# valida-xyz/valida

Measured on NVIDIA H100. Metric: trace rows/sec proven (Fibonacci), higher is better.
Workload: dtype u32 (BabyBear, 31-bit modular) + ext5

## Files before the change

valida_b200/csrc/keccak.cuh:

```cuda
#pragma once
#include <cstdint>
#include <cuda_runtime.h>

namespace kk {

__constant__ uint2 RC[24] = {
    {0x00000001u, 0x00000000u}, {0x00008082u, 0x00000000u}, {0x0000808au, 0x80000000u}, {0x80008000u, 0x80000000u},
    {0x0000808bu, 0x00000000u}, {0x80000001u, 0x00000000u}, {0x80008081u, 0x80000000u}, {0x00008009u, 0x80000000u},
    {0x0000008au, 0x00000000u}, {0x00000088u, 0x00000000u}, {0x80008009u, 0x00000000u}, {0x8000000au, 0x00000000u},
    {0x8000808bu, 0x00000000u}, {0x0000008bu, 0x80000000u}, {0x00008089u, 0x80000000u}, {0x00008003u, 0x80000000u},
    {0x00008002u, 0x80000000u}, {0x00000080u, 0x80000000u}, {0x0000800au, 0x00000000u}, {0x8000000au, 0x80000000u},
    {0x80008081u, 0x80000000u}, {0x00008080u, 0x80000000u}, {0x80000001u, 0x00000000u}, {0x80008008u, 0x80000000u}};

__constant__ uint32_t POW2[32] = {1u << 0, 1u << 1, 1u << 2, 1u << 3, 1u << 4, 1u << 5, 1u << 6, 1u << 7, 1u << 8, 1u << 9, 1u << 10, 1u << 11,
                                  1u << 12, 1u << 13, 1u << 14, 1u << 15, 1u << 16, 1u << 17, 1u << 18, 1u << 19, 1u << 20, 1u << 21, 1u << 22,
                                  1u << 23, 1u << 24, 1u << 25, 1u << 26, 1u << 27, 1u << 28, 1u << 29, 1u << 30, 1u << 31};

template <int M> __device__ __forceinline__ uint2 rol_small(uint2 a) {
    const uint32_t p = POW2[M];
    uint32_t wlo, whi, nlo, nhi;
    asm("{\n\t.reg .u64 w;\n\tmul.wide.u32 w, %4, %6;\n\tmov.b64 {%0, %1}, w;\n\tmad.lo.u32 %3, %5, %6, %1;\n\tmad.hi.u32 %2, %5, %6, %0;\n\t}"
        : "=&r"(wlo), "=&r"(whi), "=r"(nlo), "=r"(nhi) : "r"(a.x), "r"(a.y), "r"(p));
    return make_uint2(nlo, nhi);
}
#ifndef KK_FMA_ROT_MASK
#define KK_FMA_ROT_MASK 0ull
#endif
template <int M> __device__ __forceinline__ uint2 rol_shf(uint2 a) {
    return make_uint2(__funnelshift_l(a.y, a.x, M), __funnelshift_l(a.x, a.y, M));
}
template <int N> __device__ __forceinline__ uint2 rol(uint2 a) {
    if (N == 0) return a;
    if (N == 32) return make_uint2(a.y, a.x);
    constexpr int M = (N & 31) ? (N & 31) : 1;
    const uint2 b = N < 32 ? a : make_uint2(a.y, a.x);
    if ((KK_FMA_ROT_MASK >> N) & 1ull) return rol_small<M>(b);
    return rol_shf<M>(b);
}
__device__ __forceinline__ uint2 x2(uint2 a, uint2 b) { return make_uint2(a.x ^ b.x, a.y ^ b.y); }
__device__ __forceinline__ uint2 x3(uint2 a, uint2 b, uint2 c) { return make_uint2(a.x ^ b.x ^ c.x, a.y ^ b.y ^ c.y); }
__device__ __forceinline__ uint2 x5(uint2 a, uint2 b, uint2 c, uint2 d, uint2 e) { return make_uint2(a.x ^ b.x ^ c.x ^ d.x ^ e.x, a.y ^ b.y ^ c.y ^ d.y ^ e.y); }
__device__ __forceinline__ uint2 chi(uint2 a, uint2 b, uint2 c) { return make_uint2(a.x ^ (~b.x & c.x), a.y ^ (~b.y & c.y)); }

__device__ __forceinline__ void keccak_round(uint2 A[25], const uint2 rc) {
    uint2 C0 = x5(A[0], A[5], A[10], A[15], A[20]);
    uint2 C1 = x5(A[1], A[6], A[11], A[16], A[21]);
    uint2 C2 = x5(A[2], A[7], A[12], A[17], A[22]);
    uint2 C3 = x5(A[3], A[8], A[13], A[18], A[23]);
    uint2 C4 = x5(A[4], A[9], A[14], A[19], A[24]);
    const uint2 R0 = rol<1>(C1), R1 = rol<1>(C2), R2 = rol<1>(C3), R3 = rol<1>(C4), R4 = rol<1>(C0);
    uint2 B0 = x3(A[0], C4, R0);
    uint2 B10 = rol<1>(x3(A[1], C0, R1));
    uint2 B20 = rol<62>(x3(A[2], C1, R2));
    uint2 B5 = rol<28>(x3(A[3], C2, R3));
    uint2 B15 = rol<27>(x3(A[4], C3, R4));
    uint2 B16 = rol<36>(x3(A[5], C4, R0));
    uint2 B1 = rol<44>(x3(A[6], C0, R1));
    uint2 B11 = rol<6>(x3(A[7], C1, R2));
    uint2 B21 = rol<55>(x3(A[8], C2, R3));
    uint2 B6 = rol<20>(x3(A[9], C3, R4));
    uint2 B7 = rol<3>(x3(A[10], C4, R0));
    uint2 B17 = rol<10>(x3(A[11], C0, R1));
    uint2 B2 = rol<43>(x3(A[12], C1, R2));
    uint2 B12 = rol<25>(x3(A[13], C2, R3));
    uint2 B22 = rol<39>(x3(A[14], C3, R4));
    uint2 B23 = rol<41>(x3(A[15], C4, R0));
    uint2 B8 = rol<45>(x3(A[16], C0, R1));
    uint2 B18 = rol<15>(x3(A[17], C1, R2));
    uint2 B3 = rol<21>(x3(A[18], C2, R3));
    uint2 B13 = rol<8>(x3(A[19], C3, R4));
    uint2 B14 = rol<18>(x3(A[20], C4, R0));
    uint2 B24 = rol<2>(x3(A[21], C0, R1));
    uint2 B9 = rol<61>(x3(A[22], C1, R2));
    uint2 B19 = rol<56>(x3(A[23], C2, R3));
    uint2 B4 = rol<14>(x3(A[24], C3, R4));
    A[0] = chi(B0, B1, B2); A[1] = chi(B1, B2, B3); A[2] = chi(B2, B3, B4); A[3] = chi(B3, B4, B0); A[4] = chi(B4, B0, B1);
    A[5] = chi(B5, B6, B7); A[6] = chi(B6, B7, B8); A[7] = chi(B7, B8, B9); A[8] = chi(B8, B9, B5); A[9] = chi(B9, B5, B6);
    A[10] = chi(B10, B11, B12); A[11] = chi(B11, B12, B13); A[12] = chi(B12, B13, B14); A[13] = chi(B13, B14, B10); A[14] = chi(B14, B10, B11);
    A[15] = chi(B15, B16, B17); A[16] = chi(B16, B17, B18); A[17] = chi(B17, B18, B19); A[18] = chi(B18, B19, B15); A[19] = chi(B19, B15, B16);
    A[20] = chi(B20, B21, B22); A[21] = chi(B21, B22, B23); A[22] = chi(B22, B23, B24); A[23] = chi(B23, B24, B20); A[24] = chi(B24, B20, B21);
    A[0].x ^= rc.x; A[0].y ^= rc.y;
}

template <bool FIRST, bool LAST>
__device__ __forceinline__ void keccak_f_peeled(uint2 A[25]) {
    if (FIRST) keccak_round(A, make_uint2(0x00000001u, 0x00000000u));
#pragma unroll 1
    for (int round = FIRST ? 1 : 0; round < (LAST ? 23 : 24); round++) keccak_round(A, RC[round]);
    if (LAST) keccak_round(A, make_uint2(0x80008008u, 0x80000000u));
}
__device__ __forceinline__ void keccak_f(uint2 A[25]) { keccak_f_peeled<false, false>(A); }

}
```

valida_b200/csrc/merkle.cu:

```cuda
#include "ctx.h"
#include "keccak.cuh"
#include "merkle.h"
#include <algorithm>
#include <cstdlib>
#include <numeric>

namespace {

constexpr int RATE_WORDS = 34;

template <bool SHORT = false, class Fetch>
__device__ __forceinline__ void keccak256_words(const uint32_t nwords, Fetch fetch, uint32_t out[8]) {
    uint2 A[25];
#pragma unroll
    for (int i = 0; i < 25; i++) A[i] = make_uint2(0, 0);
    uint32_t nblocks = nwords / RATE_WORDS + 1;
    if (SHORT) {
#pragma unroll
        for (int i = 0; i < RATE_WORDS / 2; i++) {
            const uint32_t g0 = 2 * i, g1 = g0 + 1;
            uint32_t w0 = g0 < nwords ? fetch(g0) : (g0 == nwords ? 1u : 0u);
            uint32_t w1 = g1 < nwords ? fetch(g1) : (g1 == nwords ? 1u : 0u);
            if (i == RATE_WORDS / 2 - 1) w1 ^= 0x80000000u;
            A[i] = make_uint2(w0, w1);
        }
        kk::keccak_f_peeled<true, true>(A);
        out[0] = A[0].x; out[1] = A[0].y; out[2] = A[1].x; out[3] = A[1].y;
        out[4] = A[2].x; out[5] = A[2].y; out[6] = A[3].x; out[7] = A[3].y;
        return;
    }
    for (uint32_t b = 0; b < nblocks; b++) {
        uint32_t base = b * RATE_WORDS;
#pragma unroll
        for (int i = 0; i < RATE_WORDS / 2; i++) {
            uint32_t g0 = base + 2 * i, g1 = g0 + 1;
            uint32_t w0 = g0 < nwords ? fetch(g0) : (g0 == nwords ? 1u : 0u);
            uint32_t w1 = g1 < nwords ? fetch(g1) : (g1 == nwords ? 1u : 0u);
            if (i == RATE_WORDS / 2 - 1 && b == nblocks - 1) w1 ^= 0x80000000u;
            A[i].x ^= w0; A[i].y ^= w1;
        }
        if (b == nblocks - 1) kk::keccak_f_peeled<false, true>(A); else kk::keccak_f(A);
    }
    out[0] = A[0].x; out[1] = A[0].y; out[2] = A[1].x; out[3] = A[1].y;
    out[4] = A[2].x; out[5] = A[2].y; out[6] = A[3].x; out[7] = A[3].y;
}

__device__ __forceinline__ uint32_t wrap_mod_p(uint32_t w) {
    w = bb::umin32(w, w - bb::P);
    return bb::umin32(w, w - bb::P);
}

__global__ void __launch_bounds__(128) leaf_hash_kernel(const uint32_t* const* __restrict__ colptr, uint32_t nwords, uint64_t row0, uint64_t nrows, uint32_t* __restrict__ digests) {
    uint64_t r = (uint64_t)blockIdx.x * blockDim.x + threadIdx.x;
    if (r >= nrows) return;
    r += row0;
    uint32_t d[8];
    keccak256_words(nwords, [&](uint32_t i) { return bb::from_monty(__ldg(colptr[i] + r)); }, d);
    uint4* o = reinterpret_cast<uint4*>(digests + r * 8);
    o[0] = make_uint4(wrap_mod_p(d[0]), wrap_mod_p(d[1]), wrap_mod_p(d[2]), wrap_mod_p(d[3]));
    o[1] = make_uint4(wrap_mod_p(d[4]), wrap_mod_p(d[5]), wrap_mod_p(d[6]), wrap_mod_p(d[7]));
}

__device__ __forceinline__ void compress_pair(const uint32_t l[8], const uint32_t r[8], uint32_t out[8]) {
    uint32_t d[8];
    keccak256_words<true>(16, [&](uint32_t i) { return i < 8 ? l[i] : r[i - 8]; }, d);
#pragma unroll
    for (int i = 0; i < 8; i++) out[i] = wrap_mod_p(d[i]);
}

__global__ void __launch_bounds__(128) compress_layer_kernel(const uint32_t* __restrict__ prev, const uint32_t* __restrict__ inject, uint64_t i0, uint64_t n_next, uint32_t* __restrict__ next) {
    uint64_t i = (uint64_t)blockIdx.x * blockDim.x + threadIdx.x;
    if (i >= n_next) return;
    i += i0;
    uint32_t l[8], r[8], o[8];
    const uint4* p = reinterpret_cast<const uint4*>(prev + i * 16);
    uint4 a = __ldg(p), b = __ldg(p + 1), c = __ldg(p + 2), d = __ldg(p + 3);
    l[0] = a.x; l[1] = a.y; l[2] = a.z; l[3] = a.w; l[4] = b.x; l[5] = b.y; l[6] = b.z; l[7] = b.w;
    r[0] = c.x; r[1] = c.y; r[2] = c.z; r[3] = c.w; r[4] = d.x; r[5] = d.y; r[6] = d.z; r[7] = d.w;
    compress_pair(l, r, o);
    if (inject) {
        const uint4* q = reinterpret_cast<const uint4*>(inject + i * 8);
        uint4 e = __ldg(q), f = __ldg(q + 1);
        uint32_t t[8] = {e.x, e.y, e.z, e.w, f.x, f.y, f.z, f.w};
        uint32_t o2[8];
        compress_pair(o, t, o2);
#pragma unroll
        for (int k = 0; k < 8; k++) o[k] = o2[k];
    }
    uint4* w = reinterpret_cast<uint4*>(next + i * 8);
    w[0] = make_uint4(o[0], o[1], o[2], o[3]);
    w[1] = make_uint4(o[4], o[5], o[6], o[7]);
}

__constant__ uint8_t WK_ROT[25] = {0, 1, 62, 28, 27, 36, 44, 6, 55, 20, 3, 10, 43, 25, 39, 41, 45, 15, 21, 8, 18, 2, 61, 56, 14};
struct WarpKeccak {
    uint32_t rot, col[4], dm, dp, pi, c1, c2, lane;
    __device__ __forceinline__ void init(uint32_t lane_) {
        lane = lane_;
        const uint32_t t = lane < 25 ? lane : 0, x = t % 5, y = t / 5;
        rot = WK_ROT[t];
#pragma unroll
        for (int k = 0; k < 4; k++) col[k] = (t + 5 * (k + 1)) % 25;
        dm = (x + 4) % 5 + 5 * y; dp = (x + 1) % 5 + 5 * y;
        pi = (x + 3 * y) % 5 + 5 * x;
        c1 = (x + 1) % 5 + 5 * y; c2 = (x + 2) % 5 + 5 * y;
    }
    static __device__ __forceinline__ uint2 sh(uint2 v, uint32_t src) { return make_uint2(__shfl_sync(0xffffffffu, v.x, src), __shfl_sync(0xffffffffu, v.y, src)); }
    __device__ __forceinline__ void permute(uint2& a) const {
#pragma unroll 1
        for (int round = 0; round < 24; round++) {
            uint2 p = a;
#pragma unroll
            for (int k = 0; k < 4; k++) { const uint2 o = sh(a, col[k]); p.x ^= o.x; p.y ^= o.y; }
            const uint2 pm = sh(p, dm), pp = sh(p, dp);
            a.x ^= pm.x ^ __funnelshift_l(pp.y, pp.x, 1); a.y ^= pm.y ^ __funnelshift_l(pp.x, pp.y, 1);
            uint32_t lo = a.x, hi = a.y;
            if (rot & 32) { const uint32_t tmp = lo; lo = hi; hi = tmp; }
            uint2 b = make_uint2(__funnelshift_l(hi, lo, rot & 31), __funnelshift_l(lo, hi, rot & 31));
            b = sh(b, pi);
            const uint2 b1 = sh(b, c1), b2 = sh(b, c2);
            a.x = b.x ^ (~b1.x & b2.x); a.y = b.y ^ (~b1.y & b2.y);
            if (lane == 0) { const uint2 rc = kk::RC[round]; a.x ^= rc.x; a.y ^= rc.y; }
            if (lane >= 25) a = make_uint2(0, 0);
        }
    }
    __device__ __forceinline__ uint2 compress(uint2 words) const {
        uint2 a = lane < 8 ? words : lane == 8 ? make_uint2(1u, 0u) : lane == 16 ? make_uint2(0u, 0x80000000u) : make_uint2(0u, 0u);
        permute(a);
        return make_uint2(wrap_mod_p(a.x), wrap_mod_p(a.y));
    }
};

constexpr int TAIL_SUB = 256, TAIL_THREADS = 512, TAIL_MAX_LEVELS = 9, TAIL_WARP_NODES = 32;
struct TailParams {
    const uint32_t* prev_v;
    uint32_t* next_v[TAIL_MAX_LEVELS];
    const uint32_t* inj_v[TAIL_MAX_LEVELS];
    uint64_t first_begin;
    uint32_t sub;
    uint32_t levels;
};
__global__ void __maxnreg__(80) tree_tail_kernel(const __grid_constant__ TailParams p) {
    __shared__ uint4 buf_a[2 * TAIL_SUB * 2];
    __shared__ uint4 buf_b[TAIL_SUB * 2];
    const uint64_t node0 = p.first_begin + (uint64_t)blockIdx.x * p.sub;
    {
        const uint4* src = reinterpret_cast<const uint4*>(p.prev_v + 2 * node0 * 8);
        for (uint32_t i = threadIdx.x; i < 4 * p.sub; i += TAIL_THREADS) buf_a[i] = __ldg(src + i);
    }
    __syncthreads();
    WarpKeccak wk;
    wk.init(threadIdx.x & 31);
    uint4* cur = buf_a; uint4* nxt = buf_b;
    for (uint32_t k = 0; k < p.levels; k++) {
        const uint32_t n = p.sub >> k;
        const uint64_t base = node0 >> k;
        if (n > TAIL_WARP_NODES) {
            for (uint32_t t = threadIdx.x; t < n; t += TAIL_THREADS) {
                const uint4 a = cur[4 * t], b = cur[4 * t + 1], c = cur[4 * t + 2], d = cur[4 * t + 3];
                uint32_t l[8] = {a.x, a.y, a.z, a.w, b.x, b.y, b.z, b.w}, r[8] = {c.x, c.y, c.z, c.w, d.x, d.y, d.z, d.w}, o[8];
                compress_pair(l, r, o);
                if (p.inj_v[k]) {
                    const uint4* q = reinterpret_cast<const uint4*>(p.inj_v[k] + (base + t) * 8);
                    const uint4 e = __ldg(q), f = __ldg(q + 1);
                    uint32_t tt[8] = {e.x, e.y, e.z, e.w, f.x, f.y, f.z, f.w}, o2[8];
                    compress_pair(o, tt, o2);
#pragma unroll
                    for (int i = 0; i < 8; i++) o[i] = o2[i];
                }
                const uint4 w0 = make_uint4(o[0], o[1], o[2], o[3]), w1 = make_uint4(o[4], o[5], o[6], o[7]);
                nxt[2 * t] = w0; nxt[2 * t + 1] = w1;
                uint4* g = reinterpret_cast<uint4*>(p.next_v[k] + (base + t) * 8);
                g[0] = w0; g[1] = w1;
            }
        } else {
            const uint32_t lane = threadIdx.x & 31;
            for (uint32_t t = threadIdx.x >> 5; t < n; t += TAIL_THREADS / 32) {
                const uint2* in = reinterpret_cast<const uint2*>(cur + 4 * t);
                uint2 dg = wk.compress(lane < 8 ? in[lane] : make_uint2(0, 0));
                if (p.inj_v[k]) {
                    const uint2* q = reinterpret_cast<const uint2*>(p.inj_v[k] + (base + t) * 8);
                    const uint2 w = lane < 4 ? dg : (lane < 8 ? __ldg(q + (lane - 4)) : make_uint2(0, 0));
                    dg = wk.compress(w);
                }
                if (lane < 4) {
                    reinterpret_cast<uint2*>(nxt + 2 * t)[lane] = dg;
                    reinterpret_cast<uint2*>(p.next_v[k] + (base + t) * 8)[lane] = dg;
                }
            }
        }
        __syncthreads();
        uint4* tmp = cur; cur = nxt; nxt = tmp;
    }
}

__global__ void __launch_bounds__(128) fri_leaf_hash_kernel(const uint32_t* __restrict__ v, uint64_t cs, uint64_t i0, uint64_t npairs, uint32_t* __restrict__ digests) {
    uint64_t i = (uint64_t)blockIdx.x * blockDim.x + threadIdx.x;
    if (i >= npairs) return;
    i += i0;
    uint32_t w[10];
#pragma unroll
    for (int l = 0; l < 5; l++) {
        uint2 t = __ldg(reinterpret_cast<const uint2*>(v + (uint64_t)l * cs + 2 * i));
        w[l] = bb::from_monty(t.x); w[5 + l] = bb::from_monty(t.y);
    }
    uint32_t d[8];
    keccak256_words<true>(10, [&](uint32_t k) { return w[k]; }, d);
    uint4* o = reinterpret_cast<uint4*>(digests + i * 8);
    o[0] = make_uint4(wrap_mod_p(d[0]), wrap_mod_p(d[1]), wrap_mod_p(d[2]), wrap_mod_p(d[3]));
    o[1] = make_uint4(wrap_mod_p(d[4]), wrap_mod_p(d[5]), wrap_mod_p(d[6]), wrap_mod_p(d[7]));
}

}

struct LayerPlan { uint64_t len, cbegin, ccount, sbegin, scount; bool gather; };
static std::vector<LayerPlan> plan_tree(const vgpu_ctx* ctx, uint64_t leaves, bool split) {
    const uint64_t G = split ? (uint64_t)ctx->comm_size : 1, r = split ? (uint64_t)ctx->comm_rank : 0;
    std::vector<LayerPlan> plan;
    for (uint64_t len = leaves; len >= 1; len >>= 1) {
        LayerPlan p{};
        p.len = len;
        if (G > 1 && len >= G) { p.ccount = len / G; p.cbegin = r * p.ccount; } else { p.cbegin = 0; p.ccount = len; }
        if (G > 1 && len > G) { p.sbegin = p.cbegin; p.scount = p.ccount; } else { p.sbegin = 0; p.scount = len; }
        p.gather = G > 1 && len == G;
        plan.push_back(p);
        if (len == 1) break;
    }
    return plan;
}
static int32_t alloc_tree(vgpu_ctx* ctx, const std::vector<LayerPlan>& plan, VgTree* t) {
    uint64_t total = 0;
    for (auto& p : plan) total += p.scount;
    VG_TRY(vg_alloc(ctx, (void**)&t->digests, total * 32));
    t->layer_ptr.clear(); t->layer_len.clear(); t->layer_begin.clear(); t->layer_count.clear();
    uint32_t* at = t->digests;
    for (auto& p : plan) { t->layer_ptr.push_back(at); t->layer_len.push_back(p.len); t->layer_begin.push_back(p.sbegin); t->layer_count.push_back(p.scount); at += p.scount * 8; }
    return 0;
}
void vg_tree_free(vgpu_ctx* ctx, VgTree* t) { vg_free(ctx, t->digests); t->digests = nullptr; }

static int32_t hash_rows(vgpu_ctx* ctx, const std::vector<const vgpu_dmat*>& mats, uint64_t row0, uint64_t nrows, uint32_t* digests_v) {
    std::vector<const uint32_t*> cols;
    for (auto* m : mats) {
        if (m->dist == VG_ROWS && (row0 < m->row0 || row0 + nrows > m->row0 + m->h)) VG_FAIL(ctx, "commit: rows [%llu, +%llu) are not in this rank's shard", (unsigned long long)row0, (unsigned long long)nrows);
        for (uint64_t c = 0; c < m->w; c++) cols.push_back(m->d + c * m->col_stride - m->row0);
    }
    const uint32_t** dcols = nullptr;
    VG_TRY(vg_alloc(ctx, (void**)&dcols, cols.size() * sizeof(void*)));
    VG_CUDA(ctx, cudaMemcpyAsync(dcols, cols.data(), cols.size() * sizeof(void*), cudaMemcpyHostToDevice, ctx->stream));
    {
        KScope ks(ctx, KC_LEAF_HASH, (double)nrows * (4.0 * cols.size() + 32.0));
        leaf_hash_kernel<<<(unsigned)((nrows + 127) / 128), 128, 0, ctx->stream>>>(dcols, (uint32_t)cols.size(), row0, nrows, digests_v);
    }
    VG_LAUNCH_CHECK(ctx);
    vg_free(ctx, dcols);
    return 0;
}

constexpr uint64_t TAIL_FUSE = 1u << 15;
template <class Inject>
static int32_t build_upper_layers(vgpu_ctx* ctx, const std::vector<LayerPlan>& plan, VgTree* t, uint32_t* inject_buf, Inject inject) {
    if (plan[0].gather) VG_TRY(vg_comm_allgather_inplace(ctx, t->layer_ptr[0], 8));
    static const bool fuse = [] { const char* e = getenv("VGPU_TREE_TAIL"); return !e || atoi(e) != 0; }();
    size_t lvl = 1;
    while (lvl < plan.size()) {
        const LayerPlan& p = plan[lvl];
        const uint32_t* prev_v = t->layer_ptr[lvl - 1] - plan[lvl - 1].sbegin * 8;
        if (fuse && p.ccount <= TAIL_FUSE) {
            TailParams tp{};
            tp.prev_v = prev_v; tp.first_begin = p.cbegin;
            tp.sub = (uint32_t)std::min<uint64_t>(TAIL_SUB, p.ccount);
            uint32_t n = 0;
            uint32_t* inj_at = inject_buf;
            double bytes = 0;
            while (n < TAIL_MAX_LEVELS && lvl + n < plan.size() && (tp.sub >> n) >= 1) {
                const LayerPlan& q = plan[lvl + n];
                if (q.ccount != (p.ccount >> n) || q.cbegin != (p.cbegin >> n)) break;
                tp.next_v[n] = t->layer_ptr[lvl + n] - q.sbegin * 8;
                tp.inj_v[n] = nullptr;
                if (inject_buf) {
                    uint32_t* buf_v = inj_at - q.cbegin * 8;
                    bool have = false;
                    VG_TRY(inject(lvl + n, q, buf_v, &have));
                    if (have) { tp.inj_v[n] = buf_v; inj_at += q.ccount * 8; }
                }
                bytes += (double)q.ccount * (tp.inj_v[n] ? 128.0 : 96.0);
                n++;
                if (q.gather) break;
            }
            tp.levels = n;
            {
                KScope ks(ctx, KC_COMPRESS, bytes);
                tree_tail_kernel<<<(unsigned)(p.ccount / tp.sub), TAIL_THREADS, 0, ctx->stream>>>(tp);
            }
            VG_LAUNCH_CHECK(ctx);
            lvl += n;
            if (plan[lvl - 1].gather) VG_TRY(vg_comm_allgather_inplace(ctx, t->layer_ptr[lvl - 1], 8));
            continue;
        }
        uint32_t* next_v = t->layer_ptr[lvl] - p.sbegin * 8;
        const uint32_t* inj_v = nullptr;
        if (inject_buf) {
            uint32_t* buf_v = inject_buf - p.cbegin * 8;
            bool have = false;
            VG_TRY(inject(lvl, p, buf_v, &have));
            if (have) inj_v = buf_v;
        }
        {
            KScope ks(ctx, KC_COMPRESS, (double)p.ccount * (inj_v ? 128.0 : 96.0));
            compress_layer_kernel<<<(unsigned)((p.ccount + 127) / 128), 128, 0, ctx->stream>>>(prev_v, inj_v, p.cbegin, p.ccount, next_v);
        }
        VG_LAUNCH_CHECK(ctx);
        if (p.gather) VG_TRY(vg_comm_allgather_inplace(ctx, t->layer_ptr[lvl], 8));
        lvl++;
    }
    return 0;
}

int32_t vg_fri_layer_commit(vgpu_ctx* ctx, const uint32_t* v, uint64_t cs, uint64_t npairs, bool v_is_shard, VgTree* tree, uint32_t root_out[8]) {
    const std::vector<LayerPlan> plan = plan_tree(ctx, npairs, v_is_shard);
    VG_TRY(alloc_tree(ctx, plan, tree));
    const LayerPlan& l0 = plan[0];
    {
        const uint32_t* v_v = v_is_shard ? v - 2 * l0.cbegin : v;
        KScope ks(ctx, KC_FRI_LEAF, (double)l0.ccount * 72.0);
        fri_leaf_hash_kernel<<<(unsigned)((l0.ccount + 127) / 128), 128, 0, ctx->stream>>>(v_v, cs, l0.cbegin, l0.ccount, tree->layer_ptr[0] - l0.sbegin * 8);
    }
    VG_LAUNCH_CHECK(ctx);
    VG_TRY(build_upper_layers(ctx, plan, tree, nullptr, [](size_t, const LayerPlan&, uint32_t*, bool*) { return 0; }));
    VG_CUDA(ctx, cudaMemcpyAsync(root_out, tree->layer_ptr.back(), 32, cudaMemcpyDeviceToHost, ctx->stream));
    VG_CUDA(ctx, cudaStreamSynchronize(ctx->stream));
    return 0;
}

int32_t vg_merkle_build(vgpu_ctx* ctx, vgpu_prover_data* pd, const std::vector<uint64_t>& heights,
                        const std::function<int32_t(const std::vector<size_t>&)>& need) {
    size_t n = heights.size();
    if (!n) VG_FAIL(ctx, "commit: no matrices");
    std::vector<size_t> order(n);
    std::iota(order.begin(), order.end(), 0);
    std::stable_sort(order.begin(), order.end(), [&](size_t a, size_t b) { return heights[a] > heights[b]; });
    uint64_t max_h = heights[order[0]];
    if (max_h & (max_h - 1)) VG_FAIL(ctx, "commit: heights must be powers of two");
    pd->max_height = max_h;
    const std::vector<LayerPlan> plan = plan_tree(ctx, max_h, vg_split_rows(ctx, max_h));
    VG_TRY(alloc_tree(ctx, plan, &pd->tree));
    size_t pos = 0;
    std::vector<size_t> idx;
    std::vector<const vgpu_dmat*> group;
    auto take = [&](uint64_t height) -> int32_t {
        idx.clear(); group.clear();
        while (pos < n && heights[order[pos]] == height) idx.push_back(order[pos++]);
        if (idx.empty()) return 0;
        if (need) VG_TRY(need(idx));
        for (size_t i : idx) {
            if (!pd->ldes[i] || pd->ldes[i]->gh != height) VG_FAIL(ctx, "commit: matrix %zu was not extended to height %llu", i, (unsigned long long)height);
            group.push_back(pd->ldes[i]);
        }
        return 0;
    };
    VG_TRY(take(max_h));
    VG_TRY(hash_rows(ctx, group, plan[0].cbegin, plan[0].ccount, pd->tree.layer_ptr[0] - plan[0].sbegin * 8));
    uint32_t* inject_buf = nullptr;
    if (pos < n) {
        const uint64_t c1 = plan.size() > 1 ? plan[1].ccount : 1;
        VG_TRY(vg_alloc(ctx, (void**)&inject_buf, (c1 <= 2 * TAIL_FUSE ? 2 * c1 : c1) * 32));
    }
    int32_t rc = build_upper_layers(ctx, plan, &pd->tree, inject_buf, [&](size_t, const LayerPlan& p, uint32_t* buf_v, bool* have) -> int32_t {
        VG_TRY(take(p.len));
        *have = !group.empty();
        if (*have) VG_TRY(hash_rows(ctx, group, p.cbegin, p.ccount, buf_v));
        return 0;
    });
    if (inject_buf) vg_free(ctx, inject_buf);
    if (rc) return rc;
    if (pos != n) VG_FAIL(ctx, "commit: a matrix height does not match any tree layer");
    VG_CUDA(ctx, cudaMemcpyAsync(pd->root, pd->tree.layer_ptr.back(), 32, cudaMemcpyDeviceToHost, ctx->stream));
    VG_CUDA(ctx, cudaStreamSynchronize(ctx->stream));
    return 0;
}
```

Before: 24.55 million.

## Specialize leaf hash for few blocks, use lop3 xor3, split tail tree loop

Adds a templated leaf-hash kernel for rows that fit in one or two Keccak rate blocks. It takes the column pointers as a __grid_constant__ kernel parameter, which removes the device allocation, host-to-device copy and free of the pointer table, and it fully unrolls absorption. Keccak's three-way XOR is written as a single lop3 instruction. The tail tree kernel is split into a thread-per-node phase followed by a warp-cooperative phase, so WarpKeccak is initialized only when it is needed. The larger parameter struct and unrolled code may raise register pressure.

```diff
diff --git a/valida_b200/csrc/keccak.cuh b/valida_b200/csrc/keccak.cuh
--- a/valida_b200/csrc/keccak.cuh
+++ b/valida_b200/csrc/keccak.cuh
@@ -38,7 +38,12 @@
     return rol_shf<M>(b);
 }
 __device__ __forceinline__ uint2 x2(uint2 a, uint2 b) { return make_uint2(a.x ^ b.x, a.y ^ b.y); }
-__device__ __forceinline__ uint2 x3(uint2 a, uint2 b, uint2 c) { return make_uint2(a.x ^ b.x ^ c.x, a.y ^ b.y ^ c.y); }
+__device__ __forceinline__ uint32_t xor3(uint32_t a, uint32_t b, uint32_t c) {
+    uint32_t d;
+    asm("lop3.b32 %0, %1, %2, %3, 0x96;" : "=r"(d) : "r"(a), "r"(b), "r"(c));
+    return d;
+}
+__device__ __forceinline__ uint2 x3(uint2 a, uint2 b, uint2 c) { return make_uint2(xor3(a.x, b.x, c.x), xor3(a.y, b.y, c.y)); }
 __device__ __forceinline__ uint2 x5(uint2 a, uint2 b, uint2 c, uint2 d, uint2 e) { return make_uint2(a.x ^ b.x ^ c.x ^ d.x ^ e.x, a.y ^ b.y ^ c.y ^ d.y ^ e.y); }
 __device__ __forceinline__ uint2 chi(uint2 a, uint2 b, uint2 c) { return make_uint2(a.x ^ (~b.x & c.x), a.y ^ (~b.y & c.y)); }
 
diff --git a/valida_b200/csrc/merkle.cu b/valida_b200/csrc/merkle.cu
--- a/valida_b200/csrc/merkle.cu
+++ b/valida_b200/csrc/merkle.cu
@@ -59,6 +59,32 @@
     uint4* o = reinterpret_cast<uint4*>(digests + r * 8);
     o[0] = make_uint4(wrap_mod_p(d[0]), wrap_mod_p(d[1]), wrap_mod_p(d[2]), wrap_mod_p(d[3]));
     o[1] = make_uint4(wrap_mod_p(d[4]), wrap_mod_p(d[5]), wrap_mod_p(d[6]), wrap_mod_p(d[7]));
+}
+
+constexpr int LEAF_NB_MAX = 2;
+struct LeafCols { const uint32_t* col[LEAF_NB_MAX * RATE_WORDS]; };
+template <int NB>
+__global__ void __launch_bounds__(128) leaf_hash_kernel_blocks(const __grid_constant__ LeafCols c, uint32_t nwords, uint64_t row0, uint64_t nrows, uint32_t* __restrict__ digests) {
+    uint64_t r = (uint64_t)blockIdx.x * blockDim.x + threadIdx.x;
+    if (r >= nrows) return;
+    r += row0;
+    uint2 A[25];
+#pragma unroll
+    for (int i = 0; i < 25; i++) A[i] = make_uint2(0, 0);
+#pragma unroll
+    for (int b = 0; b < NB; b++) {
+#pragma unroll
+        for (int i = 0; i < RATE_WORDS; i++) {
+            const uint32_t g = b * RATE_WORDS + i;
+            uint32_t w = (b < NB - 1 || g < nwords) ? bb::from_monty(__ldg(c.col[g] + r)) : (g == nwords ? 1u : 0u);
+            if (b == NB - 1 && i == RATE_WORDS - 1) w ^= 0x80000000u;
+            if (i & 1) A[i / 2].y ^= w; else A[i / 2].x ^= w;
+        }
+        if (b == 0) kk::keccak_f_peeled<true, NB == 1>(A); else kk::keccak_f_peeled<false, true>(A);
+    }
+    uint4* o = reinterpret_cast<uint4*>(digests + r * 8);
+    o[0] = make_uint4(wrap_mod_p(A[0].x), wrap_mod_p(A[0].y), wrap_mod_p(A[1].x), wrap_mod_p(A[1].y));
+    o[1] = make_uint4(wrap_mod_p(A[2].x), wrap_mod_p(A[2].y), wrap_mod_p(A[3].x), wrap_mod_p(A[3].y));
 }
 
 __device__ __forceinline__ void compress_pair(const uint32_t l[8], const uint32_t r[8], uint32_t out[8]) {
@@ -149,44 +175,49 @@
         for (uint32_t i = threadIdx.x; i < 4 * p.sub; i += TAIL_THREADS) buf_a[i] = __ldg(src + i);
     }
     __syncthreads();
-    WarpKeccak wk;
-    wk.init(threadIdx.x & 31);
     uint4* cur = buf_a; uint4* nxt = buf_b;
-    for (uint32_t k = 0; k < p.levels; k++) {
+    uint32_t k = 0;
+    for (; k < p.levels && (p.sub >> k) > TAIL_WARP_NODES; k++) {
         const uint32_t n = p.sub >> k;
         const uint64_t base = node0 >> k;
-        if (n > TAIL_WARP_NODES) {
-            for (uint32_t t = threadIdx.x; t < n; t += TAIL_THREADS) {
-                const uint4 a = cur[4 * t], b = cur[4 * t + 1], c = cur[4 * t + 2], d = cur[4 * t + 3];
-                uint32_t l[8] = {a.x, a.y, a.z, a.w, b.x, b.y, b.z, b.w}, r[8] = {c.x, c.y, c.z, c.w, d.x, d.y, d.z, d.w}, o[8];
-                compress_pair(l, r, o);
-                if (p.inj_v[k]) {
-                    const uint4* q = reinterpret_cast<const uint4*>(p.inj_v[k] + (base + t) * 8);
-                    const uint4 e = __ldg(q), f = __ldg(q + 1);
-                    uint32_t tt[8] = {e.x, e.y, e.z, e.w, f.x, f.y, f.z, f.w}, o2[8];
-                    compress_pair(o, tt, o2);
-#pragma unroll
-                    for (int i = 0; i < 8; i++) o[i] = o2[i];
-                }
-                const uint4 w0 = make_uint4(o[0], o[1], o[2], o[3]), w1 = make_uint4(o[4], o[5], o[6], o[7]);
-                nxt[2 * t] = w0; nxt[2 * t + 1] = w1;
-                uint4* g = reinterpret_cast<uint4*>(p.next_v[k] + (base + t) * 8);
-                g[0] = w0; g[1] = w1;
+        for (uint32_t t = threadIdx.x; t < n; t += TAIL_THREADS) {
+            const uint4 a = cur[4 * t], b = cur[4 * t + 1], c = cur[4 * t + 2], d = cur[4 * t + 3];
+            uint32_t l[8] = {a.x, a.y, a.z, a.w, b.x, b.y, b.z, b.w}, r[8] = {c.x, c.y, c.z, c.w, d.x, d.y, d.z, d.w}, o[8];
+            compress_pair(l, r, o);
+            if (p.inj_v[k]) {
+                const uint4* q = reinterpret_cast<const uint4*>(p.inj_v[k] + (base + t) * 8);
+                const uint4 e = __ldg(q), f = __ldg(q + 1);
+                uint32_t tt[8] = {e.x, e.y, e.z, e.w, f.x, f.y, f.z, f.w}, o2[8];
+                compress_pair(o, tt, o2);
+#pragma unroll
+                for (int i = 0; i < 8; i++) o[i] = o2[i];
             }
-        } else {
-            const uint32_t lane = threadIdx.x & 31;
-            for (uint32_t t = threadIdx.x >> 5; t < n; t += TAIL_THREADS / 32) {
-                const uint2* in = reinterpret_cast<const uint2*>(cur + 4 * t);
-                uint2 dg = wk.compress(lane < 8 ? in[lane] : make_uint2(0, 0));
-                if (p.inj_v[k]) {
-                    const uint2* q = reinterpret_cast<const uint2*>(p.inj_v[k] + (base + t) * 8);
-                    const uint2 w = lane < 4 ? dg : (lane < 8 ? __ldg(q + (lane - 4)) : make_uint2(0, 0));
-                    dg = wk.compress(w);
-                }
-                if (lane < 4) {
-                    reinterpret_cast<uint2*>(nxt + 2 * t)[lane] = dg;
-                    reinterpret_cast<uint2*>(p.next_v[k] + (base + t) * 8)[lane] = dg;
-                }
+            const uint4 w0 = make_uint4(o[0], o[1], o[2], o[3]), w1 = make_uint4(o[4], o[5], o[6], o[7]);
+            nxt[2 * t] = w0; nxt[2 * t + 1] = w1;
+            uint4* g = reinterpret_cast<uint4*>(p.next_v[k] + (base + t) * 8);
+            g[0] = w0; g[1] = w1;
+        }
+        __syncthreads();
+        uint4* tmp = cur; cur = nxt; nxt = tmp;
+    }
+    if (k == p.levels) return;
+    const uint32_t lane = threadIdx.x & 31;
+    WarpKeccak wk;
+    wk.init(lane);
+    for (; k < p.levels; k++) {
+        const uint32_t n = p.sub >> k;
+        const uint64_t base = node0 >> k;
+        for (uint32_t t = threadIdx.x >> 5; t < n; t += TAIL_THREADS / 32) {
+            const uint2* in = reinterpret_cast<const uint2*>(cur + 4 * t);
+            uint2 dg = wk.compress(lane < 8 ? in[lane] : make_uint2(0, 0));
+            if (p.inj_v[k]) {
+                const uint2* q = reinterpret_cast<const uint2*>(p.inj_v[k] + (base + t) * 8);
+                const uint2 w = lane < 4 ? dg : (lane < 8 ? __ldg(q + (lane - 4)) : make_uint2(0, 0));
+                dg = wk.compress(w);
+            }
+            if (lane < 4) {
+                reinterpret_cast<uint2*>(nxt + 2 * t)[lane] = dg;
+                reinterpret_cast<uint2*>(p.next_v[k] + (base + t) * 8)[lane] = dg;
             }
         }
         __syncthreads();
@@ -245,12 +276,24 @@
         if (m->dist == VG_ROWS && (row0 < m->row0 || row0 + nrows > m->row0 + m->h)) VG_FAIL(ctx, "commit: rows [%llu, +%llu) are not in this rank's shard", (unsigned long long)row0, (unsigned long long)nrows);
         for (uint64_t c = 0; c < m->w; c++) cols.push_back(m->d + c * m->col_stride - m->row0);
     }
+    const uint32_t nwords = (uint32_t)cols.size(), nblocks = nwords / RATE_WORDS + 1, grid = (uint32_t)((nrows + 127) / 128);
+    if (nblocks <= LEAF_NB_MAX) {
+        LeafCols lc{};
+        std::copy(cols.begin(), cols.end(), lc.col);
+        {
+            KScope ks(ctx, KC_LEAF_HASH, (double)nrows * (4.0 * nwords + 32.0));
+            if (nblocks == 1) leaf_hash_kernel_blocks<1><<<grid, 128, 0, ctx->stream>>>(lc, nwords, row0, nrows, digests_v);
+            else leaf_hash_kernel_blocks<2><<<grid, 128, 0, ctx->stream>>>(lc, nwords, row0, nrows, digests_v);
+        }
+        VG_LAUNCH_CHECK(ctx);
+        return 0;
+    }
     const uint32_t** dcols = nullptr;
     VG_TRY(vg_alloc(ctx, (void**)&dcols, cols.size() * sizeof(void*)));
     VG_CUDA(ctx, cudaMemcpyAsync(dcols, cols.data(), cols.size() * sizeof(void*), cudaMemcpyHostToDevice, ctx->stream));
     {
-        KScope ks(ctx, KC_LEAF_HASH, (double)nrows * (4.0 * cols.size() + 32.0));
-        leaf_hash_kernel<<<(unsigned)((nrows + 127) / 128), 128, 0, ctx->stream>>>(dcols, (uint32_t)cols.size(), row0, nrows, digests_v);
+        KScope ks(ctx, KC_LEAF_HASH, (double)nrows * (4.0 * nwords + 32.0));
+        leaf_hash_kernel<<<grid, 128, 0, ctx->stream>>>(dcols, nwords, row0, nrows, digests_v);
     }
     VG_LAUNCH_CHECK(ctx);
     vg_free(ctx, dcols);
```

After: 25.91 million, median of 6. 1.06x the previous value.
